# zzyunzhi/object-intrinsics

Hardware: AMD Instinct MI355X
Metric: rendered rays/sec (64x64 img, 128 samples/ray) + D-images/sec (higher is better)
Workload: dtype f32 via f16x3 (fp32 operands split into 2 fp16 limbs = 22 mantissa bits, 3 fp16 MFMAs per product, fp32 accumulate: 2^-22 relative per product, 1e-4 parity path); 1 GPU; C2: 1x64x64 crop per GPU, 64+64 samples/ray, 1 up-sampling step(s), Generator.forward (render + Phong maps) + ADADiscriminatorView forward; parallelism=dp1 (independent renders, no data-path collective)

## Files before the change

object-intrinsics_amd/build.py:

```python
import hashlib
import os
import subprocess
import sys

HERE = os.path.dirname(os.path.abspath(__file__))
CSRC = os.path.join(HERE, "csrc")
OUT_DIR = os.path.join(HERE, "oi_amd")
LIB = os.path.join(OUT_DIR, "liboi_hip.so")
STAMP = os.path.join(OUT_DIR, ".liboi_hip.stamp")
SOURCES = ["mlp.hip", "mlp_fwd3.hip", "mlp_fwd3b.hip", "color_head.hip", "render.hip", "disc.hip", "disc_small.hip", "disc_large.hip", "mlp_bwd.hip", "render_bwd.hip", "disc_bwd.hip", "optim.hip", "loss.hip", "mesh.hip", "relight.hip", "mesh_attr.hip", "trace.hip", "mesh_band.hip", "occlusion.hip", "trace_batch.hip", "envlight.hip", "scene.hip"]
FLAGS = ["--offload-arch=gfx950", "-O3", "-std=c++17", "-fPIC", "-Wno-unused-value"] + os.environ.get("OI_FLAGS", "").split()
EXTRA = {"mlp_fwd3.hip": ["-mllvm", "-amdgpu-mfma-vgpr-form=1"],
         "mlp_fwd3b.hip": ["-mllvm", "-amdgpu-mfma-vgpr-form=1", "-fno-slp-vectorize"],
         "mlp_bwd.hip": ["-mllvm", "-amdgpu-mfma-vgpr-form=1"]}


def _hipcc():
    for c in (os.environ.get("HIPCC"), "/opt/rocm/bin/hipcc", "hipcc"):
        if c and (os.path.isabs(c) and os.path.exists(c) or not os.path.isabs(c)):
            return c
    raise RuntimeError("hipcc not found")


def _sources():
    return [s for s in SOURCES if os.path.exists(os.path.join(CSRC, s))]


def _digest():
    h = hashlib.sha256()
    files = [os.path.join(CSRC, f) for f in sorted(os.listdir(CSRC))]
    inc = os.path.join(os.path.dirname(HERE), "include")
    files += [os.path.join(inc, f) for f in sorted(os.listdir(inc))]
    for f in files:
        with open(f, "rb") as fh:
            h.update(os.path.basename(f).encode())
# ... 37 lines not shown
```

object-intrinsics_amd/csrc/mlp_fwd3.hip:

```cpp
#include <type_traits>

#include "mlp_common.h"
#include "f3_blob.h"

namespace {

using namespace oimlp;
static_assert(oif3::FC == C && oif3::HB_SIG == H_SIG && oif3::HB_TABS_END == H_TABS_END && oif3::HB_BIAS == H_BIAS &&
              oif3::HB_WSCALE == H_WSCALE && oif3::HB_NL_SDF == NL_SDF, "f3_blob.h mirrors the packed header's offsets");

constexpr int F3_WAVES = 4;
constexpr int F3_TILE = F3_WAVES * WAVE_PTS;
using oif3::F3_FILM;
using oif3::F3_FILM_ROW;
using oif3::F3_TABS;
using oif3::F3_GMAX;
using oif3::F3_BLOB;
constexpr int F3_LDS = F3_BLOB + 2 * 65536;

typedef float Bank[16][4];
__device__ __forceinline__ float to_acc(float v) {
  float a;
  asm("v_accvgpr_write_b32 %0, %1" : "=a"(a) : "v"(v));
  return a;
}
__device__ __forceinline__ float from_acc(float a) {
  float v;
  asm("v_accvgpr_read_b32 %0, %1" : "=v"(v) : "a"(a));
  return v;
}

constexpr int F3_CU_SLOTS = 4096;
constexpr int F3_WG_SLOTS = 512;
__device__ __forceinline__ int cu_slot_id() {
  const unsigned xcc = __builtin_amdgcn_s_getreg((4 - 1) << 11 | 0 << 6 | 20);
  const unsigned cu = __builtin_amdgcn_s_getreg((8 - 1) << 11 | 8 << 6 | 4);
  return (int)(xcc * 256 + cu);
}

typedef float f32x2 __attribute__((ext_vector_type(2)));
__device__ __forceinline__ f32x2 pk_fma(f32x2 a, f32x2 b, f32x2 c) {
  return __builtin_elementwise_fma(a, b, c);
}
__device__ __forceinline__ f32x2 pk_mul(f32x2 a, f32x2 b) {
  return a * b;
}
__device__ __forceinline__ f32x2 pk_mul_s(f32x2 a, float s) {
  return a * s;
}
__device__ __forceinline__ f32x2 film_phase2(const f32x4& a, const f32x4& b, int k, float acc0, float acc1) {
  return pk_fma(f32x2{a[k], a[k + 1]}, f32x2{acc0, acc1}, f32x2{b[k], b[k + 1]});
}
__device__ __forceinline__ float max3_abs(float m, float x, float y) {
  float r;
  asm("v_max3_f32 %0, %1, |%2|, |%3|" : "=v"(r) : "v"(m), "v"(x), "v"(y));
  return r;
}

typedef unsigned Limbs[8][4];


__device__ __forceinline__ void split_limbs_normalised(const float (&act)[64], float m, float& run, Limbs& bh, Limbs& bl) {
  m = fmaxf(m, __shfl_xor(m, 32, 64));
  int eb = (__builtin_bit_cast(int, m) >> 23) & 0xff;
  eb = eb < 14 ? 14 : (eb > 254 ? 254 : eb);
  const float sc = __builtin_bit_cast(float, (267 - eb) << 23);
  run *= __builtin_bit_cast(float, (eb - 13) << 23);
#pragma unroll
  for (int s = 0; s < 8; ++s) {
#pragma unroll
    for (int d = 0; d < 4; ++d) split_pair(act[8 * s + 2 * d] * sc, act[8 * s + 2 * d + 1] * sc, bh[s][d], bl[s][d]);
    __builtin_amdgcn_sched_barrier(0);
  }
}
__device__ __forceinline__ void split_limbs(const float (&act)[64], Limbs& bh, Limbs& bl) {
#pragma unroll
  for (int s = 0; s < 8; ++s) {
#pragma unroll
    for (int d = 0; d < 4; ++d) split_pair(act[8 * s + 2 * d], act[8 * s + 2 * d + 1], bh[s][d], bl[s][d]);
    __builtin_amdgcn_sched_barrier(0);
  }
}

struct NoTail {
  __device__ __forceinline__ void operator()(int, int) const {}
};
template <class T> struct is_no_tail { static constexpr bool value = false; };
template <> struct is_no_tail<NoTail> { static constexpr bool value = true; };

constexpr int F3_ADIST = 1;
constexpr int F3_VALU_PER_MFMA = 6;
struct NoMid {
  __device__ __forceinline__ void operator()() const {}
};
template <class TAIL, class MID, class EPI>
__device__ __forceinline__ void stream_layer(const char* lds, const LayOff& y, const Limbs& bh, const Limbs& bl,
                                             f32x16 (&acc)[4], TAIL&& tail, MID&& mid, EPI&& epi) {
  constexpr bool HAS_TAIL = !is_no_tail<std::remove_cv_t<std::remove_reference_t<TAIL>>>::value;
  constexpr int AD = F3_ADIST;
  f32x4 ah[AD + 1], al[AD + 1];
#pragma unroll
  for (int i = 0; i < AD; ++i) {
    ah[i] = lds_f4(lds, i * 1024, y.wl);
    al[i] = lds_f4(lds, i * 1024, y.wh);
  }
#pragma unroll
  for (int t = 0; t < 4; ++t) {
#pragma unroll
    for (int r = 0; r < 16; ++r) acc[t][r] = 0.f;
#pragma unroll
    for (int s = 0; s < 8; ++s) {
      const int cur = t * 8 + s, nxt = cur + AD;
      if (nxt < 32) {
        ah[nxt % (AD + 1)] = lds_f4(lds, nxt * 1024, y.wl);
        al[nxt % (AD + 1)] = lds_f4(lds, nxt * 1024, y.wh);
      }
      int npairs = 0;
      if (t == 0) {
        if (HAS_TAIL && s < 6) {
          constexpr int first[7] = {0, 2, 3, 4, 6, 7, 8};
          for (int rp = first[s]; rp < first[s + 1]; ++rp) tail(3, rp);
          npairs = first[s + 1] - first[s];
        }
      } else {
        epi(t - 1, s);
        npairs = 1;
      }
      const int ci = cur % (AD + 1);
      const f16x8 wh = __builtin_bit_cast(f16x8, ah[ci]);
      const f16x8 wl = __builtin_bit_cast(f16x8, al[ci]);
      const u32x4 uh = {bh[s][0], bh[s][1], bh[s][2], bh[s][3]}, ul = {bl[s][0], bl[s][1], bl[s][2], bl[s][3]};
      const f16x8 vh = __builtin_bit_cast(f16x8, uh);
      const f16x8 vl = __builtin_bit_cast(f16x8, ul);
      acc[t] = __builtin_amdgcn_mfma_f32_32x32x16_f16(wl, vh, acc[t], 0, 0, 0);
      acc[t] = __builtin_amdgcn_mfma_f32_32x32x16_f16(wh, vl, acc[t], 0, 0, 0);
      acc[t] = __builtin_amdgcn_mfma_f32_32x32x16_f16(wh, vh, acc[t], 0, 0, 0);
      if (npairs >= 1) {
#pragma unroll
        for (int q = 0; q < 2; ++q) {
          __builtin_amdgcn_sched_group_barrier(0x008, 1, 0);
          if (npairs <= 1) __builtin_amdgcn_sched_group_barrier(0x002, F3_VALU_PER_MFMA, 0);
          else __builtin_amdgcn_sched_group_barrier(0x002, 2 * F3_VALU_PER_MFMA, 0);
        }
        __builtin_amdgcn_sched_group_barrier(0x008, 1, 0);
      }
      __builtin_amdgcn_sched_barrier(0);
    }
    if (t == 0) {
      mid();
      __builtin_amdgcn_sched_barrier(0);
    }
  }
}
template <class EPI>
__device__ __forceinline__ void run_tail(EPI&& epi) {
#pragma unroll
  for (int rp = 0; rp < 8; ++rp) {
    epi(3, rp);
    if (rp & 1) __builtin_amdgcn_sched_barrier(0);
  }
}

#ifdef OI_F3_PROF
__device__ unsigned long long oi_prof3[16];
#define F3_T(i)                                                  \
  do {                                                           \
    const unsigned long long t_ = __builtin_readcyclecounter();  \
    pacc[i] += t_ - tprev;                                       \
    tprev = t_;                                                  \
  } while (0)
#else
#define F3_T(i)
#endif

template <bool FAST>
__global__ void __launch_bounds__(64 * F3_WAVES) __attribute__((amdgpu_waves_per_eu(1, 1)))
sdf_mlp_full3_kernel(const float* __restrict__ pts, const char* __restrict__ packed, const float* __restrict__ gamma,
                     const float* __restrict__ beta, float* __restrict__ sdf_out, float* __restrict__ grad_out,
                     float* __restrict__ rgb_out, float* __restrict__ feat_out, char* __restrict__ scratch,
                     const char* __restrict__ blob, long long n_per_elem) {
  extern __shared__ __attribute__((aligned(16))) char lds[];
  constexpr int LB = 65536;
#ifdef OI_F3_PROF
// ... 21 lines not shown
    valid = local < n_per_elem;
    return (long long)e * n_per_elem + (valid ? local : n_per_elem - 1);
  };

  FwdScratch<false> ws;
  {
    long long wg = (long long)e * gridDim.x + blockIdx.x;
    if ((long long)gridDim.x * gridDim.y > F3_WG_SLOTS) wg = cu_slot_id();
    ws.rs = __builtin_amdgcn_make_buffer_rsrc(scratch + (wg * F3_WAVES + wave) * 16384ll, 0, 16384, 0x00020000);
  }

  __amdgpu_buffer_rsrc_t feat_rs;
  int feat_off;
  {
    const long long base_pt = (long long)e * n_per_elem + (long long)blockIdx.x * F3_TILE + wave * WAVE_PTS;
    const long long left = n_per_elem - ((long long)blockIdx.x * F3_TILE + wave * WAVE_PTS);
    const int npts = feat_out == nullptr ? 0 : (left >= WAVE_PTS ? WAVE_PTS : (left > 0 ? (int)left : 0));
    feat_rs = __builtin_amdgcn_make_buffer_rsrc(feat_out + base_pt * C, 0, npts * C * 4, 0x00020000);
    feat_off = j * C * 4 + 16 * h;
  }

  const __amdgpu_buffer_rsrc_t img_rs =
      __builtin_amdgcn_make_buffer_rsrc(const_cast<char*>(mats), 0, NMAT * LB, 0x00020000);
  auto prefetch = [&](int pos) {
    const int m = pos < 7 ? pos : (pos < 12 ? 20 - pos : (pos < 14 ? pos - 12 : (pos < 16 ? 22 - pos : 14)));
#pragma unroll
    for (int q = 0; q < LB / 4096 / F3_WAVES; ++q) {
      const int c = (wave * (LB / 4096 / F3_WAVES) + q) * 4096;
      auto* dst = (__attribute__((address_space(3))) void*)(lds + F3_BLOB + (pos & 1) * LB + c);
      __builtin_amdgcn_raw_ptr_buffer_load_lds(img_rs, dst, 16, o.l16, m * LB + c, 0, 0);
      __builtin_amdgcn_raw_ptr_buffer_load_lds(img_rs, dst, 16, o.l16, m * LB + c, 1024, 0);
      __builtin_amdgcn_raw_ptr_buffer_load_lds(img_rs, dst, 16, o.l16, m * LB + c, 2048, 0);
      __builtin_amdgcn_raw_ptr_buffer_load_lds(img_rs, dst, 16, o.l16, m * LB + c, 3072, 0);
    }
  };
  auto lay = [&](int pos) {
    LayOff y;
    y.wl = o.l16 + F3_BLOB + (pos & 1) * LB;
    y.wh = y.wl + 32768;
    y.wq = 0;
    y.f16 = 0;
    return y;
  };
  auto film_base = [&](int l) { return o.h16 + F3_FILM + l * F3_FILM_ROW; };

  float px, py, pz;
  {
    bool valid;
    const long long pt = point_of(valid);
    px = pts[pt * 3 + 0], py = pts[pt * 3 + 1], pz = pts[pt * 3 + 2];
  }
  {
    const __amdgpu_buffer_rsrc_t blob_rs =
        __builtin_amdgcn_make_buffer_rsrc(const_cast<char*>(blob + (size_t)e * F3_BLOB), 0, F3_BLOB, 0x00020000);
#pragma unroll
    for (int q = 0; q < (F3_BLOB / 1024 + F3_WAVES - 1) / F3_WAVES; ++q) {
      const int c = q * F3_WAVES + wave;
      if (c < F3_BLOB / 1024)
        __builtin_amdgcn_raw_ptr_buffer_load_lds(blob_rs, (__attribute__((address_space(3))) void*)(lds + c * 1024), 16, o.l16,
                                                 c * 1024, 0, 0);
    }
  }
  prefetch(0);
  asm volatile("s_waitcnt vmcnt(%0) lgkmcnt(0)\n\ts_barrier" ::"n"(LB / 1024 / F3_WAVES) : "memory");
#ifdef OI_F3_PROF
  unsigned long long pacc[8] = {0, 0, 0, 0, 0, 0, 0, 0};
  unsigned long long tprev = __builtin_readcyclecounter();
  const unsigned long long tstart = tprev;
  pacc[4] = tstart - t_entry;
#endif
  float act[64];
  f32x16 acc[4];
  Limbs AH, AL, BH, BL;
  Bank P0, P1, P2, P3;
  struct Rows {
    f32x4 a, b, c, d;
  } rw[2];
  f32x4 fv;
  float run = 1.f, vmax = 0.f, sdf_part = 0.f;

  auto reduce = [&](float phi) { return FAST ? phi : __builtin_amdgcn_fractf(phi); };
  auto ld = [&](int imm, int base) { return lds_f4(lds, imm, base); };
#define ROW_A(FB, G) ld(grp_f0(G) * 4, FB)
#define ROW_B(FB, G) ld((C + grp_f0(G)) * 4, FB)
#define ROW_G(FB, G) ld((2 * C + grp_f0(G)) * 4, FB)
#define ROW_SIG(G) ld(F3_TABS + (H_SIG + grp_f0(G)) * 4, o.h16)

#define OI_PARK(BANK) [&](int g, int k, float r) { BANK[g][k] = to_acc(r); }
  auto no_park = [](int, int, float) {};

  auto layer0 = [&](Limbs& NH, Limbs& NL, auto&& park) {
    const int fb = film_base(0);
#pragma unroll
    for (int g = 0; g < 16; ++g) {
      const f32x4 a4 = ROW_A(fb, g), b4 = ROW_B(fb, g);
      float sn[4];
#pragma unroll
      for (int k = 0; k < 4; ++k) {
        const f32x4 w = lds_f4(lds, F3_TABS + H_TAB0 * 4 + (grp_f0(g) + k) * 16, o.h64);
        const float u = fmaf(pz, w[2], fmaf(py, w[1], px * w[0]));
        const float r = reduce(fmaf(a4[k], u, b4[k]));
        sn[k] = __builtin_amdgcn_sinf(r);
        park(g, k, r);
      }
      split_pair(sn[0], sn[1], NH[g >> 1][2 * (g & 1)], NL[g >> 1][2 * (g & 1)]);
      split_pair(sn[2], sn[3], NH[g >> 1][2 * (g & 1) + 1], NL[g >> 1][2 * (g & 1) + 1]);
      if (g & 1) __builtin_amdgcn_sched_barrier(0);
    }
  };

#define OI_FWD_EPI(FB, NH, NL, PARK, NEXT)                                                                 \
  [&](int tb, int rp) {                                                                                    \
    const int g = tb * 4 + (rp >> 1), k = 2 * (rp & 1);                                                    \
    Rows& R = rw[g & 1];                                                                                   \
    if (k == 0) {                                                                                          \
      if (g < 15) {                                                                                        \
        rw[(g + 1) & 1].a = ROW_A(FB, g + 1);                                                              \
        rw[(g + 1) & 1].b = ROW_B(FB, g + 1);                                                              \
      } else {                                                                                             \
        NEXT;                                                                                              \
      }                                                                                                    \
    }                                                                                                      \
    const f32x2 ph = film_phase2(R.a, R.b, k, acc[tb][2 * rp], acc[tb][2 * rp + 1]);                 \
    const float r0 = reduce(ph[0]), r1 = reduce(ph[1]);                                                    \
    PARK(g, k, r0);                                                                                        \
    PARK(g, k + 1, r1);                                                                                    \
    split_pair(__builtin_amdgcn_sinf(r0), __builtin_amdgcn_sinf(r1), NH[2 * tb + (rp >> 2)][rp & 3],       \
               NL[2 * tb + (rp >> 2)][rp & 3]);                                                            \
  }
  float sg = 1.f;
  auto pow2_for = [&](float U) {
    int eb = (__builtin_bit_cast(int, U) >> 23) & 0xff;
    eb = eb < 15 ? 15 : (eb > 253 ? 253 : eb);
    run *= __builtin_bit_cast(float, (eb - 14) << 23);
    sg = __builtin_bit_cast(float, (268 - eb) << 23);
  };
  const float* gmax = reinterpret_cast<const float*>(lds + F3_GMAX);
#define OI_REV_MID(L)                                                          \
  [&]() {                                                                      \
    const float m = fmaxf(vmax, __shfl_xor(vmax, 32, 64));                     \
    pow2_for(m * (hdr[H_BOUND + 6 + (L)] * gmax[(L)-1]));                      \
    vmax = 0.f;                                                                \
  }
#define OI_REV_EPI(FB, BANK, NH, NL, NEXT)                                                                 \
  [&](int tb, int rp) {                                                                                    \
    const int g = tb * 4 + (rp >> 1), k = 2 * (rp & 1);                                                    \
    Rows& R = rw[g & 1];                                                                                   \
    if (k == 0) {                                                                                          \
      if (g < 15) {                                                                                        \
        rw[(g + 1) & 1].c = ROW_G(FB, g + 1);                                                              \
      } else {                                                                                             \
        NEXT;                                                                                              \
      }                                                                                                    \
    }                                                                                                      \
    const f32x2 cs = {__builtin_amdgcn_cosf(from_acc(BANK[g][k])), __builtin_amdgcn_cosf(from_acc(BANK[g][k + 1]))};                     \
    const f32x2 v = pk_mul(pk_mul_s(f32x2{acc[tb][2 * rp], acc[tb][2 * rp + 1]}, sg),                \
                           pk_mul(f32x2{R.c[k], R.c[k + 1]}, cs));                                         \
    vmax = max3_abs(vmax, v[0], v[1]);                                                                     \
    split_pair(v[0], v[1], NH[2 * tb + (rp >> 2)][rp & 3], NL[2 * tb + (rp >> 2)][rp & 3]);                \
  }

  const LayOff y1 = lay(0), y2 = lay(1), y3 = lay(2), y4 = lay(3), y5 = lay(4), y6 = lay(5), y7 = lay(6);
  const int F0 = film_base(0), F1 = film_base(1), F2 = film_base(2), F3 = film_base(3), F4 = film_base(4),
            F5 = film_base(5), F6 = film_base(6), F7 = film_base(7), F8 = film_base(8), F9 = film_base(9);
#define NEXT_AB(FB) (rw[0].a = ROW_A(FB, 0), rw[0].b = ROW_B(FB, 0))
#define NEXT_G(FB) (rw[0].c = ROW_G(FB, 0))

  layer0(AH, AL, no_park);
  NEXT_AB(F1);
  F3_T(0);
  ring_sync();
  F3_T(2);
  prefetch(1);
  auto park0 = OI_PARK(P0);
  auto park1 = OI_PARK(P1);
  auto park2 = OI_PARK(P2);
  auto park3 = OI_PARK(P3);
  auto e1 = OI_FWD_EPI(F1, BH, BL, no_park, NEXT_AB(F2));
  stream_layer(lds, y1, AH, AL, acc, NoTail(), NoMid(), e1);
  F3_T(1);
  ring_sync();
  F3_T(2);
  prefetch(2);
  auto e2 = OI_FWD_EPI(F2, AH, AL, no_park, NEXT_AB(F3));
  stream_layer(lds, y2, BH, BL, acc, e1, NoMid(), e2);
  F3_T(1);
  ring_sync();
  F3_T(2);
  prefetch(3);
  auto e3 = OI_FWD_EPI(F3, BH, BL, park0, NEXT_AB(F4));
  stream_layer(lds, y3, AH, AL, acc, e2, NoMid(), e3);
  F3_T(1);
  ring_sync();
  F3_T(2);
  prefetch(4);
  auto e4 = OI_FWD_EPI(F4, AH, AL, park1, NEXT_AB(F5));
  stream_layer(lds, y4, BH, BL, acc, e3, NoMid(), e4);
  F3_T(1);
  ring_sync();
  F3_T(2);
  prefetch(5);
  auto e5 = OI_FWD_EPI(F5, BH, BL, park2, NEXT_AB(F6));
  stream_layer(lds, y5, AH, AL, acc, e4, NoMid(), e5);
  F3_T(1);
  ring_sync();
  F3_T(2);
  prefetch(6);
  auto e6 = OI_FWD_EPI(F6, AH, AL, park3,
                       (NEXT_AB(F7), rw[0].c = ROW_A(F9, 0), rw[0].d = ROW_SIG(0)));
  stream_layer(lds, y6, BH, BL, acc, e5, NoMid(), e6);
  F3_T(1);
  ring_sync();
  F3_T(2);
  prefetch(7);
  pow2_for(gmax[9] * 2.0f);
  const float sg7 = sg;
  auto e7 = [&](int tb, int rp) {
    const int g = tb * 4 + (rp >> 1), k = 2 * (rp & 1);
    Rows& R = rw[g & 1];
    if (k == 0) {
      if (g < 15) {
        Rows& N = rw[(g + 1) & 1];
        N.a = ROW_A(F7, g + 1);
        N.b = ROW_B(F7, g + 1);
        N.c = ROW_A(F9, g + 1);
        N.d = ROW_SIG(g + 1);
      } else {
        NEXT_G(F6);
      }
    }
    const f32x2 ph = film_phase2(R.a, R.b, k, acc[tb][2 * rp], acc[tb][2 * rp + 1]);
    f32x2 cs;
#pragma unroll
    for (int i = 0; i < 2; ++i) {
      const float r = reduce(ph[i]);
      const float sn = __builtin_amdgcn_sinf(r);
      fv[k + i] = sn;
      sdf_part = fmaf(sn, R.d[k + i], sdf_part);
      cs[i] = __builtin_amdgcn_cosf(r);
    }
    const f32x2 v = pk_mul(pk_mul_s(f32x2{R.c[k], R.c[k + 1]}, sg7), cs);
    vmax = max3_abs(vmax, v[0], v[1]);
    split_pair(v[0], v[1], BH[2 * tb + (rp >> 2)][rp & 3], BL[2 * tb + (rp >> 2)][rp & 3]);
    if (k == 2) {
      ws.store(0, g, o, fv);
      __builtin_amdgcn_raw_buffer_store_b128(__builtin_bit_cast(u32x4, fv), feat_rs, feat_off + grp_f0(g) * 4, 0, 0);
    }
  };
  stream_layer(lds, y7, AH, AL, acc, e6, NoMid(), e7);
  F3_T(1);
  ring_sync();
  F3_T(2);
  prefetch(8);

  auto r7 = OI_REV_EPI(F6, P3, AH, AL, NEXT_G(F5));
  stream_layer(lds, lay(7), BH, BL, acc, e7, OI_REV_MID(7), r7);
  {
    sdf_part += __shfl_xor(sdf_part, 32, 64);
    const float sdf_v = sdf_part + *reinterpret_cast<const float*>(lds + F3_TABS + (H_SIG + C) * 4);
    bool valid;
    const long long pt = point_of(valid);
    if (valid && h == 0) sdf_out[pt] = sdf_v;
  }
  F3_T(1);
  ring_sync();
  F3_T(2);
  prefetch(9);
  auto r6 = OI_REV_EPI(F5, P2, BH, BL, NEXT_G(F4));
  stream_layer(lds, lay(8), AH, AL, acc, r7, OI_REV_MID(6), r6);
  F3_T(1);
  ring_sync();
  F3_T(2);
  prefetch(10);
  auto r5 = OI_REV_EPI(F4, P1, AH, AL, NEXT_G(F3));
  stream_layer(lds, lay(9), BH, BL, acc, r6, OI_REV_MID(5), r5);
  F3_T(1);
  ring_sync();
  F3_T(2);
  prefetch(11);
  auto r4 = OI_REV_EPI(F3, P0, BH, BL, (void)0);
  stream_layer(lds, lay(10), AH, AL, acc, r5, OI_REV_MID(4), r4);
  F3_T(1);
  ring_sync();
  F3_T(2);
  prefetch(12);
  float one = 1.0f;
  asm volatile("" : "+v"(one));
  auto pg3 = [&](int tb, int rp) {
    const int g = tb * 4 + (rp >> 1), k = 2 * (rp & 1);
    const f32x2 a = pk_mul_s(f32x2{acc[tb][2 * rp], acc[tb][2 * rp + 1]}, one);
    vmax = max3_abs(vmax, a[0], a[1]);
    P0[g][k] = to_acc(a[0]);
    P0[g][k + 1] = to_acc(a[1]);
  };
  stream_layer(lds, lay(11), BH, BL, acc, r4, [&]() { vmax = 0.f; }, pg3);
  F3_T(1);
  ring_sync();
  F3_T(2);
  prefetch(13);
  run_tail(pg3);
  F3_T(3);

  const LayOff z1 = lay(12), z2 = lay(13);
  NEXT_AB(F1);
  layer0(AH, AL, park1);
  F3_T(0);
  auto f1 = OI_FWD_EPI(F1, BH, BL, park2, (NEXT_AB(F2), NEXT_G(F2)));
  stream_layer(lds, z1, AH, AL, acc, NoTail(), NoMid(), f1);
  F3_T(1);
  ring_sync();
  F3_T(2);
  prefetch(14);
  pow2_for(fmaxf(vmax, __shfl_xor(vmax, 32, 64)) * gmax[2]);
  vmax = 0.f;
  const float sg2 = sg;
  auto f2 = [&](int tb, int rp) {
    const int g = tb * 4 + (rp >> 1), k = 2 * (rp & 1);
    Rows& R = rw[g & 1];
    if (k == 0) {
      if (g < 15) {
        Rows& N = rw[(g + 1) & 1];
        N.a = ROW_A(F2, g + 1);
        N.b = ROW_B(F2, g + 1);
        N.c = ROW_G(F2, g + 1);
      } else {
        NEXT_G(F1);
      }
    }
    const f32x2 ph = film_phase2(R.a, R.b, k, acc[tb][2 * rp], acc[tb][2 * rp + 1]);
    const f32x2 cs = {__builtin_amdgcn_cosf(reduce(ph[0])), __builtin_amdgcn_cosf(reduce(ph[1]))};
    const f32x2 v = pk_mul(pk_mul_s(f32x2{from_acc(P0[g][k]), from_acc(P0[g][k + 1])}, sg2), pk_mul(f32x2{R.c[k], R.c[k + 1]}, cs));
    vmax = max3_abs(vmax, v[0], v[1]);
    split_pair(v[0], v[1], AH[2 * tb + (rp >> 2)][rp & 3], AL[2 * tb + (rp >> 2)][rp & 3]);
  };
  stream_layer(lds, z2, BH, BL, acc, f1, NoMid(), f2);
  F3_T(1);
  ring_sync();
  F3_T(2);
  prefetch(15);

  auto r2 = OI_REV_EPI(F1, P2, BH, BL, NEXT_G(F0));
  stream_layer(lds, lay(14), AH, AL, acc, f2, OI_REV_MID(2), r2);
  F3_T(1);
  ring_sync();
  F3_T(2);
  prefetch(16);
  auto r1 = [&](int tb, int rp) {
    const int g = tb * 4 + (rp >> 1), k = 2 * (rp & 1);
    Rows& R = rw[g & 1];
    if (k == 0 && g < 15) rw[(g + 1) & 1].c = ROW_G(F0, g + 1);
    const f32x2 cs = {__builtin_amdgcn_cosf(from_acc(P1[g][k])), __builtin_amdgcn_cosf(from_acc(P1[g][k + 1]))};
    const f32x2 v = pk_mul(f32x2{acc[tb][2 * rp], acc[tb][2 * rp + 1]}, pk_mul(f32x2{R.c[k], R.c[k + 1]}, cs));
    act[4 * g + k] = v[0];
    act[4 * g + k + 1] = v[1];
  };
  stream_layer(lds, lay(15), BH, BL, acc, r2, [&]() {}, r1);
  F3_T(1);
  run_tail(r1);
  F3_T(3);
  f32x4 fback[16];
#pragma unroll
  for (int g = 0; g < 16; ++g) fback[g] = ws.load(0, g, o);
  float gx = 0.f, gy = 0.f, gz = 0.f;
#pragma unroll
  for (int g = 0; g < 16; ++g) {
#pragma unroll
    for (int k = 0; k < 4; ++k) {
      const f32x4 w = lds_f4(lds, F3_TABS + H_TAB0 * 4 + (grp_f0(g) + k) * 16, o.h64);
      const float v = act[4 * g + k];
      gx = fmaf(v, w[0], gx);
      gy = fmaf(v, w[1], gy);
      gz = fmaf(v, w[2], gz);
    }
    if (g & 1) __builtin_amdgcn_sched_barrier(0);
  }
  gx += __shfl_xor(gx, 32, 64);
  gy += __shfl_xor(gy, 32, 64);
  gz += __shfl_xor(gz, 32, 64);
  gx *= run;
  gy *= run;
  gz *= run;
  bool valid;
  const long long pt = point_of(valid);
  if (valid && h == 0) {
    grad_out[pt * 3 + 0] = gx;
    grad_out[pt * 3 + 1] = gy;
    grad_out[pt * 3 + 2] = gz;
  }

  {
    ring_sync();
#pragma unroll
    for (int g = 0; g < 16; ++g)
#pragma unroll
      for (int k = 0; k < 4; ++k) act[4 * g + k] = fback[g][k];
    const LayOff yc = lay(16);
    const float cs3 = 1.0f / hdr[H_WSCALE + 14];
    const float vx = gx * cs3, vy = gy * cs3, vz = gz * cs3;
    float r0 = 0.f, r1 = 0.f, r2 = 0.f;
    f32x4 w0, w1, w2;
    split_limbs(act, AH, AL);
    NEXT_AB(F8);
    auto ec = [&](int tb, int rp) {
      const int g = tb * 4 + (rp >> 1), k = 2 * (rp & 1);
      Rows& R = rw[g & 1];
      if (k == 0) {
        if (g < 15) {
          rw[(g + 1) & 1].a = ROW_A(F8, g + 1);
          rw[(g + 1) & 1].b = ROW_B(F8, g + 1);
        }
        w0 = lds_f4(lds, F3_TABS + (H_RGB + 0 * C + grp_f0(g)) * 4, o.h16);
        w1 = lds_f4(lds, F3_TABS + (H_RGB + 1 * C + grp_f0(g)) * 4, o.h16);
        w2 = lds_f4(lds, F3_TABS + (H_RGB + 2 * C + grp_f0(g)) * 4, o.h16);
      }
#pragma unroll
      for (int i = 0; i < 2; ++i) {
        const f32x4 w = lds_f4(lds, F3_TABS + H_TABV * 4 + (grp_f0(g) + k + i) * 16, o.h64);
        const float u = acc[tb][2 * rp + i] + fmaf(vz, w[2], fmaf(vy, w[1], vx * w[0]));
        const float sn = __builtin_amdgcn_sinf(reduce(fmaf(R.a[k + i], u, R.b[k + i])));
        r0 = fmaf(sn, w0[k + i], r0);
        r1 = fmaf(sn, w1[k + i], r1);
        r2 = fmaf(sn, w2[k + i], r2);
      }
    };
    F3_T(5);
    stream_layer(lds, yc, AH, AL, acc, NoTail(), NoMid(), ec);
    F3_T(1);
    run_tail(ec);
    F3_T(3);
    r0 += __shfl_xor(r0, 32, 64);
    r1 += __shfl_xor(r1, 32, 64);
    r2 += __shfl_xor(r2, 32, 64);
    if (valid && h == 0 && rgb_out != nullptr) {
      const float* brgb = reinterpret_cast<const float*>(lds + F3_TABS + (H_RGB + 3 * C) * 4);
      rgb_out[pt * 3 + 0] = oi::sigmoidf_(r0 + brgb[0]);
      rgb_out[pt * 3 + 1] = oi::sigmoidf_(r1 + brgb[1]);
      rgb_out[pt * 3 + 2] = oi::sigmoidf_(r2 + brgb[2]);
    }
  }
#ifdef OI_F3_PROF
  F3_T(5);
  if (lane == 0) {
    for (int i = 0; i < 6; ++i) atomicAdd(&oi_prof3[i], pacc[i]);
    atomicAdd(&oi_prof3[6], __builtin_readcyclecounter() - tstart);
    atomicAdd(&oi_prof3[7], 1ull);
    atomicAdd(&oi_prof3[8], __builtin_readcyclecounter() - t_entry);
    atomicAdd(&oi_prof3[9], __builtin_amdgcn_s_memrealtime() - rt_entry);
  }
#endif
#undef OI_PARK
#undef OI_FWD_EPI
#undef OI_REV_EPI
#undef OI_REV_MID
#undef NEXT_AB
#undef NEXT_G
#undef ROW_A
#undef ROW_B
#undef ROW_G
#undef ROW_SIG
}

__global__ void __launch_bounds__(128) film_blob_f3_kernel(const char* __restrict__ packed, const float* __restrict__ gamma,
                                                           const float* __restrict__ beta, char* __restrict__ blob) {
  __shared__ float red[8];
  const int e = blockIdx.x, l = blockIdx.y, tid = threadIdx.x;
  const float* hdr = reinterpret_cast<const float*>(packed);
  float* out = reinterpret_cast<float*>(blob + (size_t)e * F3_BLOB);
  const float gm = tid < C ? gamma[((size_t)e * 9 + l) * C + tid] : 0.f, bt = tid < C ? beta[((size_t)e * 9 + l) * C + tid] : 0.f;
  oif3::blob_layer(hdr, out, l, tid, gm, bt, red);
}

size_t full3_slot_bytes(int B, long long n_per_elem) {
  const long long wgs = (long long)B * oi::cdiv(n_per_elem, F3_TILE);
// ... 78 lines not shown
```

Measured before the change: 3.556 million rays/s.

## Interleave weight DMA and split epilogues into MFMA gaps in fused SIREN kernel

Each layer's epilogue is split into three phases that run between the three fp16 MFMAs of every step, replacing sched_group_barrier hints with explicit sched barriers. The next layer's weight prefetch is broken into 16 pieces issued one per MFMA step inside stream_layer, instead of one burst before each layer. Packed f32x2 math is replaced by scalar fmas, SLP vectorization is disabled for this file, and point coordinates are reloaded before the second pass. The aim is to hide VALU and DMA issue behind matrix ops, at the cost of more live state (st[]) and tighter scheduling constraints.

```diff
diff --git a/object-intrinsics_amd/build.py b/object-intrinsics_amd/build.py
--- a/object-intrinsics_amd/build.py
+++ b/object-intrinsics_amd/build.py
@@ -10,7 +10,7 @@
 STAMP = os.path.join(OUT_DIR, ".liboi_hip.stamp")
 SOURCES = ["mlp.hip", "mlp_fwd3.hip", "mlp_fwd3b.hip", "color_head.hip", "render.hip", "disc.hip", "disc_small.hip", "disc_large.hip", "mlp_bwd.hip", "render_bwd.hip", "disc_bwd.hip", "optim.hip", "loss.hip", "mesh.hip", "relight.hip", "mesh_attr.hip", "trace.hip", "mesh_band.hip", "occlusion.hip", "trace_batch.hip", "envlight.hip", "scene.hip"]
 FLAGS = ["--offload-arch=gfx950", "-O3", "-std=c++17", "-fPIC", "-Wno-unused-value"] + os.environ.get("OI_FLAGS", "").split()
-EXTRA = {"mlp_fwd3.hip": ["-mllvm", "-amdgpu-mfma-vgpr-form=1"],
+EXTRA = {"mlp_fwd3.hip": ["-mllvm", "-amdgpu-mfma-vgpr-form=1", "-fno-slp-vectorize"],
          "mlp_fwd3b.hip": ["-mllvm", "-amdgpu-mfma-vgpr-form=1", "-fno-slp-vectorize"],
          "mlp_bwd.hip": ["-mllvm", "-amdgpu-mfma-vgpr-form=1"]}
 
diff --git a/object-intrinsics_amd/csrc/mlp_fwd3.hip b/object-intrinsics_amd/csrc/mlp_fwd3.hip
--- a/object-intrinsics_amd/csrc/mlp_fwd3.hip
+++ b/object-intrinsics_amd/csrc/mlp_fwd3.hip
@@ -38,18 +38,11 @@
   return (int)(xcc * 256 + cu);
 }
 
-typedef float f32x2 __attribute__((ext_vector_type(2)));
-__device__ __forceinline__ f32x2 pk_fma(f32x2 a, f32x2 b, f32x2 c) {
-  return __builtin_elementwise_fma(a, b, c);
-}
-__device__ __forceinline__ f32x2 pk_mul(f32x2 a, f32x2 b) {
-  return a * b;
-}
-__device__ __forceinline__ f32x2 pk_mul_s(f32x2 a, float s) {
-  return a * s;
-}
-__device__ __forceinline__ f32x2 film_phase2(const f32x4& a, const f32x4& b, int k, float acc0, float acc1) {
-  return pk_fma(f32x2{a[k], a[k + 1]}, f32x2{acc0, acc1}, f32x2{b[k], b[k + 1]});
+struct Pair2 {
+  float x, y;
+};
+__device__ __forceinline__ Pair2 film_phase2(const f32x4& a, const f32x4& b, int k, float acc0, float acc1) {
+  return Pair2{fmaf(a[k], acc0, b[k]), fmaf(a[k + 1], acc1, b[k + 1])};
 }
 __device__ __forceinline__ float max3_abs(float m, float x, float y) {
   float r;
@@ -83,19 +76,22 @@
 }
 
 struct NoTail {
-  __device__ __forceinline__ void operator()(int, int) const {}
+  __device__ __forceinline__ void operator()(int, int, int) const {}
 };
 template <class T> struct is_no_tail { static constexpr bool value = false; };
 template <> struct is_no_tail<NoTail> { static constexpr bool value = true; };
 
 constexpr int F3_ADIST = 1;
-constexpr int F3_VALU_PER_MFMA = 6;
+constexpr int F3_DMA_PIECES = 16;
 struct NoMid {
   __device__ __forceinline__ void operator()() const {}
 };
-template <class TAIL, class MID, class EPI>
+struct NoDma {
+  __device__ __forceinline__ void operator()(int) const {}
+};
+template <class TAIL, class MID, class EPI, class DMA>
 __device__ __forceinline__ void stream_layer(const char* lds, const LayOff& y, const Limbs& bh, const Limbs& bl,
-                                             f32x16 (&acc)[4], TAIL&& tail, MID&& mid, EPI&& epi) {
+                                             f32x16 (&acc)[4], TAIL&& tail, MID&& mid, EPI&& epi, DMA&& dma) {
   constexpr bool HAS_TAIL = !is_no_tail<std::remove_cv_t<std::remove_reference_t<TAIL>>>::value;
   constexpr int AD = F3_ADIST;
   f32x4 ah[AD + 1], al[AD + 1];
@@ -111,21 +107,18 @@
 #pragma unroll
     for (int s = 0; s < 8; ++s) {
       const int cur = t * 8 + s, nxt = cur + AD;
-      if (nxt < 32) {
-        ah[nxt % (AD + 1)] = lds_f4(lds, nxt * 1024, y.wl);
-        al[nxt % (AD + 1)] = lds_f4(lds, nxt * 1024, y.wh);
-      }
-      int npairs = 0;
-      if (t == 0) {
-        if (HAS_TAIL && s < 6) {
-          constexpr int first[7] = {0, 2, 3, 4, 6, 7, 8};
-          for (int rp = first[s]; rp < first[s + 1]; ++rp) tail(3, rp);
-          npairs = first[s + 1] - first[s];
+      auto gap = [&](int q) {
+        if (t == 0) {
+          if (HAS_TAIL && s == 0) {
+            tail(3, (2 * q) / 3, (2 * q) % 3);
+            tail(3, (2 * q + 1) / 3, (2 * q + 1) % 3);
+          } else if (HAS_TAIL && s < 7) {
+            tail(3, s + 1, q);
+          }
+        } else {
+          epi(t - 1, s, q);
         }
-      } else {
-        epi(t - 1, s);
-        npairs = 1;
-      }
+      };
       const int ci = cur % (AD + 1);
       const f16x8 wh = __builtin_bit_cast(f16x8, ah[ci]);
       const f16x8 wl = __builtin_bit_cast(f16x8, al[ci]);
@@ -133,17 +126,18 @@
       const f16x8 vh = __builtin_bit_cast(f16x8, uh);
       const f16x8 vl = __builtin_bit_cast(f16x8, ul);
       acc[t] = __builtin_amdgcn_mfma_f32_32x32x16_f16(wl, vh, acc[t], 0, 0, 0);
+      if (nxt < 32) {
+        ah[nxt % (AD + 1)] = lds_f4(lds, nxt * 1024, y.wl);
+        al[nxt % (AD + 1)] = lds_f4(lds, nxt * 1024, y.wh);
+      }
+      gap(0);
+      __builtin_amdgcn_sched_barrier(0);
       acc[t] = __builtin_amdgcn_mfma_f32_32x32x16_f16(wh, vl, acc[t], 0, 0, 0);
+      if (cur < F3_DMA_PIECES) dma(cur);
+      gap(1);
+      __builtin_amdgcn_sched_barrier(0);
       acc[t] = __builtin_amdgcn_mfma_f32_32x32x16_f16(wh, vh, acc[t], 0, 0, 0);
-      if (npairs >= 1) {
-#pragma unroll
-        for (int q = 0; q < 2; ++q) {
-          __builtin_amdgcn_sched_group_barrier(0x008, 1, 0);
-          if (npairs <= 1) __builtin_amdgcn_sched_group_barrier(0x002, F3_VALU_PER_MFMA, 0);
-          else __builtin_amdgcn_sched_group_barrier(0x002, 2 * F3_VALU_PER_MFMA, 0);
-        }
-        __builtin_amdgcn_sched_group_barrier(0x008, 1, 0);
-      }
+      gap(2);
       __builtin_amdgcn_sched_barrier(0);
     }
     if (t == 0) {
@@ -154,11 +148,14 @@
 }
 template <class EPI>
 __device__ __forceinline__ void run_tail(EPI&& epi) {
+  asm volatile("; oi-exposed-begin");
 #pragma unroll
   for (int rp = 0; rp < 8; ++rp) {
-    epi(3, rp);
+#pragma unroll
+    for (int q = 0; q < 3; ++q) epi(3, rp, q);
     if (rp & 1) __builtin_amdgcn_sched_barrier(0);
   }
+  asm volatile("; oi-exposed-end");
 }
 
 #ifdef OI_F3_PROF
@@ -226,24 +223,31 @@
 
   const __amdgpu_buffer_rsrc_t img_rs =
       __builtin_amdgcn_make_buffer_rsrc(const_cast<char*>(mats), 0, NMAT * LB, 0x00020000);
+  constexpr int F3_PIECES = LB / 1024 / F3_WAVES;
+  static_assert(F3_PIECES == F3_DMA_PIECES, "stream_layer issues every piece of a wave's share");
+  auto prefetch_piece = [&](int pos, int i) {
+    const int m = pos < 7 ? pos : (pos < 12 ? 20 - pos : (pos < 14 ? pos - 12 : (pos < 16 ? 22 - pos : 14)));
+    const int c = (wave * (F3_PIECES / 4) + i / 4) * 4096;
+    auto* dst = (__attribute__((address_space(3))) void*)(lds + F3_BLOB + (pos & 1) * LB + c);
+    switch (i % 4) {
+      case 0: __builtin_amdgcn_raw_ptr_buffer_load_lds(img_rs, dst, 16, o.l16, m * LB + c, 0, 0); break;
+      case 1: __builtin_amdgcn_raw_ptr_buffer_load_lds(img_rs, dst, 16, o.l16, m * LB + c, 1024, 0); break;
+      case 2: __builtin_amdgcn_raw_ptr_buffer_load_lds(img_rs, dst, 16, o.l16, m * LB + c, 2048, 0); break;
+      default: __builtin_amdgcn_raw_ptr_buffer_load_lds(img_rs, dst, 16, o.l16, m * LB + c, 3072, 0); break;
+    }
+  };
   auto prefetch = [&](int pos) {
-    const int m = pos < 7 ? pos : (pos < 12 ? 20 - pos : (pos < 14 ? pos - 12 : (pos < 16 ? 22 - pos : 14)));
-#pragma unroll
-    for (int q = 0; q < LB / 4096 / F3_WAVES; ++q) {
-      const int c = (wave * (LB / 4096 / F3_WAVES) + q) * 4096;
-      auto* dst = (__attribute__((address_space(3))) void*)(lds + F3_BLOB + (pos & 1) * LB + c);
-      __builtin_amdgcn_raw_ptr_buffer_load_lds(img_rs, dst, 16, o.l16, m * LB + c, 0, 0);
-      __builtin_amdgcn_raw_ptr_buffer_load_lds(img_rs, dst, 16, o.l16, m * LB + c, 1024, 0);
-      __builtin_amdgcn_raw_ptr_buffer_load_lds(img_rs, dst, 16, o.l16, m * LB + c, 2048, 0);
-      __builtin_amdgcn_raw_ptr_buffer_load_lds(img_rs, dst, 16, o.l16, m * LB + c, 3072, 0);
-    }
-  };
+#pragma unroll
+    for (int i = 0; i < F3_PIECES; ++i) prefetch_piece(pos, i);
+  };
+#define OI_DMA(POS) [&](int i) { prefetch_piece(POS, i); }
   auto lay = [&](int pos) {
     LayOff y;
     y.wl = o.l16 + F3_BLOB + (pos & 1) * LB;
     y.wh = y.wl + 32768;
     y.wq = 0;
     y.f16 = 0;
+    asm volatile("" : "+v"(y.wl), "+v"(y.wh));
     return y;
   };
   auto film_base = [&](int l) { return o.h16 + F3_FILM + l * F3_FILM_ROW; };
@@ -282,6 +286,7 @@
   } rw[2];
   f32x4 fv;
   float run = 1.f, vmax = 0.f, sdf_part = 0.f;
+  float st[6];
 
   auto reduce = [&](float phi) { return FAST ? phi : __builtin_amdgcn_fractf(phi); };
   auto ld = [&](int imm, int base) { return lds_f4(lds, imm, base); };
@@ -314,23 +319,29 @@
   };
 
 #define OI_FWD_EPI(FB, NH, NL, PARK, NEXT)                                                                 \
-  [&](int tb, int rp) {                                                                                    \
+  [&](int tb, int rp, int q) {                                                                             \
     const int g = tb * 4 + (rp >> 1), k = 2 * (rp & 1);                                                    \
     Rows& R = rw[g & 1];                                                                                   \
-    if (k == 0) {                                                                                          \
-      if (g < 15) {                                                                                        \
-        rw[(g + 1) & 1].a = ROW_A(FB, g + 1);                                                              \
-        rw[(g + 1) & 1].b = ROW_B(FB, g + 1);                                                              \
-      } else {                                                                                             \
-        NEXT;                                                                                              \
+    if (q == 0) {                                                                                          \
+      const Pair2 ph = film_phase2(R.a, R.b, k, acc[tb][2 * rp], acc[tb][2 * rp + 1]);                     \
+      st[0] = reduce(ph.x);                                                                                \
+      st[1] = reduce(ph.y);                                                                                \
+    } else if (q == 1) {                                                                                   \
+      if (k == 0) {                                                                                        \
+        if (g < 15) {                                                                                      \
+          rw[(g + 1) & 1].a = ROW_A(FB, g + 1);                                                            \
+          rw[(g + 1) & 1].b = ROW_B(FB, g + 1);                                                            \
+        } else {                                                                                           \
+          NEXT;                                                                                            \
+        }                                                                                                  \
       }                                                                                                    \
+      st[2] = __builtin_amdgcn_sinf(st[0]);                                                                \
+      PARK(g, k, st[0]);                                                                                   \
+      PARK(g, k + 1, st[1]);                                                                               \
+    } else {                                                                                               \
+      split_pair(st[2], __builtin_amdgcn_sinf(st[1]), NH[2 * tb + (rp >> 2)][rp & 3],                      \
+                 NL[2 * tb + (rp >> 2)][rp & 3]);                                                          \
     }                                                                                                      \
-    const f32x2 ph = film_phase2(R.a, R.b, k, acc[tb][2 * rp], acc[tb][2 * rp + 1]);                 \
-    const float r0 = reduce(ph[0]), r1 = reduce(ph[1]);                                                    \
-    PARK(g, k, r0);                                                                                        \
-    PARK(g, k + 1, r1);                                                                                    \
-    split_pair(__builtin_amdgcn_sinf(r0), __builtin_amdgcn_sinf(r1), NH[2 * tb + (rp >> 2)][rp & 3],       \
-               NL[2 * tb + (rp >> 2)][rp & 3]);                                                            \
   }
   float sg = 1.f;
   auto pow2_for = [&](float U) {
@@ -347,24 +358,30 @@
     vmax = 0.f;                                                                \
   }
 #define OI_REV_EPI(FB, BANK, NH, NL, NEXT)                                                                 \
-  [&](int tb, int rp) {                                                                                    \
+  [&](int tb, int rp, int q) {                                                                             \
     const int g = tb * 4 + (rp >> 1), k = 2 * (rp & 1);                                                    \
     Rows& R = rw[g & 1];                                                                                   \
-    if (k == 0) {                                                                                          \
-      if (g < 15) {                                                                                        \
-        rw[(g + 1) & 1].c = ROW_G(FB, g + 1);                                                              \
-      } else {                                                                                             \
-        NEXT;                                                                                              \
+    if (q == 0) {                                                                                          \
+      st[0] = __builtin_amdgcn_cosf(from_acc(BANK[g][k]));                                                 \
+      st[1] = from_acc(BANK[g][k + 1]);                                                                    \
+    } else if (q == 1) {                                                                                   \
+      if (k == 0) {                                                                                        \
+        if (g < 15) {                                                                                      \
+          rw[(g + 1) & 1].c = ROW_G(FB, g + 1);                                                            \
+        } else {                                                                                           \
+          NEXT;                                                                                            \
+        }                                                                                                  \
       }                                                                                                    \
+      st[2] = __builtin_amdgcn_cosf(st[1]);                                                                \
+      st[3] = (acc[tb][2 * rp] * sg) * (R.c[k] * st[0]);                                                   \
+      st[4] = acc[tb][2 * rp + 1] * sg;                                                                    \
+    } else {                                                                                               \
+      const float v1 = st[4] * (R.c[k + 1] * st[2]);                                                       \
+      vmax = max3_abs(vmax, st[3], v1);                                                                    \
+      split_pair(st[3], v1, NH[2 * tb + (rp >> 2)][rp & 3], NL[2 * tb + (rp >> 2)][rp & 3]);               \
     }                                                                                                      \
-    const f32x2 cs = {__builtin_amdgcn_cosf(from_acc(BANK[g][k])), __builtin_amdgcn_cosf(from_acc(BANK[g][k + 1]))};                     \
-    const f32x2 v = pk_mul(pk_mul_s(f32x2{acc[tb][2 * rp], acc[tb][2 * rp + 1]}, sg),                \
-                           pk_mul(f32x2{R.c[k], R.c[k + 1]}, cs));                                         \
-    vmax = max3_abs(vmax, v[0], v[1]);                                                                     \
-    split_pair(v[0], v[1], NH[2 * tb + (rp >> 2)][rp & 3], NL[2 * tb + (rp >> 2)][rp & 3]);                \
-  }
-
-  const LayOff y1 = lay(0), y2 = lay(1), y3 = lay(2), y4 = lay(3), y5 = lay(4), y6 = lay(5), y7 = lay(6);
+  }
+
   const int F0 = film_base(0), F1 = film_base(1), F2 = film_base(2), F3 = film_base(3), F4 = film_base(4),
             F5 = film_base(5), F6 = film_base(6), F7 = film_base(7), F8 = film_base(8), F9 = film_base(9);
 #define NEXT_AB(FB) (rw[0].a = ROW_A(FB, 0), rw[0].b = ROW_B(FB, 0))
@@ -375,90 +392,88 @@
   F3_T(0);
   ring_sync();
   F3_T(2);
-  prefetch(1);
   auto park0 = OI_PARK(P0);
   auto park1 = OI_PARK(P1);
   auto park2 = OI_PARK(P2);
   auto park3 = OI_PARK(P3);
   auto e1 = OI_FWD_EPI(F1, BH, BL, no_park, NEXT_AB(F2));
-  stream_layer(lds, y1, AH, AL, acc, NoTail(), NoMid(), e1);
-  F3_T(1);
-  ring_sync();
-  F3_T(2);
-  prefetch(2);
+  stream_layer(lds, lay(0), AH, AL, acc, NoTail(), NoMid(), e1, OI_DMA(1));
+  F3_T(1);
+  ring_sync();
+  F3_T(2);
   auto e2 = OI_FWD_EPI(F2, AH, AL, no_park, NEXT_AB(F3));
-  stream_layer(lds, y2, BH, BL, acc, e1, NoMid(), e2);
-  F3_T(1);
-  ring_sync();
-  F3_T(2);
-  prefetch(3);
+  stream_layer(lds, lay(1), BH, BL, acc, e1, NoMid(), e2, OI_DMA(2));
+  F3_T(1);
+  ring_sync();
+  F3_T(2);
   auto e3 = OI_FWD_EPI(F3, BH, BL, park0, NEXT_AB(F4));
-  stream_layer(lds, y3, AH, AL, acc, e2, NoMid(), e3);
-  F3_T(1);
-  ring_sync();
-  F3_T(2);
-  prefetch(4);
+  stream_layer(lds, lay(2), AH, AL, acc, e2, NoMid(), e3, OI_DMA(3));
+  F3_T(1);
+  ring_sync();
+  F3_T(2);
   auto e4 = OI_FWD_EPI(F4, AH, AL, park1, NEXT_AB(F5));
-  stream_layer(lds, y4, BH, BL, acc, e3, NoMid(), e4);
-  F3_T(1);
-  ring_sync();
-  F3_T(2);
-  prefetch(5);
+  stream_layer(lds, lay(3), BH, BL, acc, e3, NoMid(), e4, OI_DMA(4));
+  F3_T(1);
+  ring_sync();
+  F3_T(2);
   auto e5 = OI_FWD_EPI(F5, BH, BL, park2, NEXT_AB(F6));
-  stream_layer(lds, y5, AH, AL, acc, e4, NoMid(), e5);
-  F3_T(1);
-  ring_sync();
-  F3_T(2);
-  prefetch(6);
+  stream_layer(lds, lay(4), AH, AL, acc, e4, NoMid(), e5, OI_DMA(5));
+  F3_T(1);
+  ring_sync();
+  F3_T(2);
   auto e6 = OI_FWD_EPI(F6, AH, AL, park3,
                        (NEXT_AB(F7), rw[0].c = ROW_A(F9, 0), rw[0].d = ROW_SIG(0)));
-  stream_layer(lds, y6, BH, BL, acc, e5, NoMid(), e6);
-  F3_T(1);
-  ring_sync();
-  F3_T(2);
-  prefetch(7);
+  stream_layer(lds, lay(5), BH, BL, acc, e5, NoMid(), e6, OI_DMA(6));
+  F3_T(1);
+  ring_sync();
+  F3_T(2);
   pow2_for(gmax[9] * 2.0f);
   const float sg7 = sg;
-  auto e7 = [&](int tb, int rp) {
+  auto e7 = [&](int tb, int rp, int q) {
     const int g = tb * 4 + (rp >> 1), k = 2 * (rp & 1);
     Rows& R = rw[g & 1];
-    if (k == 0) {
-      if (g < 15) {
-        Rows& N = rw[(g + 1) & 1];
-        N.a = ROW_A(F7, g + 1);
-        N.b = ROW_B(F7, g + 1);
-        N.c = ROW_A(F9, g + 1);
-        N.d = ROW_SIG(g + 1);
-      } else {
-        NEXT_G(F6);
+    if (q == 0) {
+      const Pair2 ph = film_phase2(R.a, R.b, k, acc[tb][2 * rp], acc[tb][2 * rp + 1]);
+      st[0] = reduce(ph.x);
+      st[1] = reduce(ph.y);
+      st[2] = __builtin_amdgcn_sinf(st[0]);
+    } else if (q == 1) {
+      if (k == 0) {
+        if (g < 15) {
+          Rows& N = rw[(g + 1) & 1];
+          N.a = ROW_A(F7, g + 1);
+          N.b = ROW_B(F7, g + 1);
+          N.c = ROW_A(F9, g + 1);
+          N.d = ROW_SIG(g + 1);
+        } else {
+          NEXT_G(F6);
+        }
       }
-    }
-    const f32x2 ph = film_phase2(R.a, R.b, k, acc[tb][2 * rp], acc[tb][2 * rp + 1]);
-    f32x2 cs;
-#pragma unroll
-    for (int i = 0; i < 2; ++i) {
-      const float r = reduce(ph[i]);
-      const float sn = __builtin_amdgcn_sinf(r);
-      fv[k + i] = sn;
-      sdf_part = fmaf(sn, R.d[k + i], sdf_part);
-      cs[i] = __builtin_amdgcn_cosf(r);
-    }
-    const f32x2 v = pk_mul(pk_mul_s(f32x2{R.c[k], R.c[k + 1]}, sg7), cs);
-    vmax = max3_abs(vmax, v[0], v[1]);
-    split_pair(v[0], v[1], BH[2 * tb + (rp >> 2)][rp & 3], BL[2 * tb + (rp >> 2)][rp & 3]);
-    if (k == 2) {
-      ws.store(0, g, o, fv);
-      __builtin_amdgcn_raw_buffer_store_b128(__builtin_bit_cast(u32x4, fv), feat_rs, feat_off + grp_f0(g) * 4, 0, 0);
-    }
-  };
-  stream_layer(lds, y7, AH, AL, acc, e6, NoMid(), e7);
-  F3_T(1);
-  ring_sync();
-  F3_T(2);
-  prefetch(8);
+      fv[k] = st[2];
+      sdf_part = fmaf(st[2], R.d[k], sdf_part);
+      asm volatile("" : "+v"(sdf_part));
+      st[3] = (R.c[k] * sg7) * __builtin_amdgcn_cosf(st[0]);
+      st[4] = __builtin_amdgcn_sinf(st[1]);
+    } else {
+      fv[k + 1] = st[4];
+      sdf_part = fmaf(st[4], R.d[k + 1], sdf_part);
+      asm volatile("" : "+v"(sdf_part));
+      const float v1 = (R.c[k + 1] * sg7) * __builtin_amdgcn_cosf(st[1]);
+      vmax = max3_abs(vmax, st[3], v1);
+      split_pair(st[3], v1, BH[2 * tb + (rp >> 2)][rp & 3], BL[2 * tb + (rp >> 2)][rp & 3]);
+      if (k == 2) {
+        ws.store(0, g, o, fv);
+        __builtin_amdgcn_raw_buffer_store_b128(__builtin_bit_cast(u32x4, fv), feat_rs, feat_off + grp_f0(g) * 4, 0, 0);
+      }
+    }
+  };
+  stream_layer(lds, lay(6), AH, AL, acc, e6, NoMid(), e7, OI_DMA(7));
+  F3_T(1);
+  ring_sync();
+  F3_T(2);
 
   auto r7 = OI_REV_EPI(F6, P3, AH, AL, NEXT_G(F5));
-  stream_layer(lds, lay(7), BH, BL, acc, e7, OI_REV_MID(7), r7);
+  stream_layer(lds, lay(7), BH, BL, acc, e7, OI_REV_MID(7), r7, OI_DMA(8));
   {
     sdf_part += __shfl_xor(sdf_part, 32, 64);
     const float sdf_v = sdf_part + *reinterpret_cast<const float*>(lds + F3_TABS + (H_SIG + C) * 4);
@@ -469,96 +484,109 @@
   F3_T(1);
   ring_sync();
   F3_T(2);
-  prefetch(9);
   auto r6 = OI_REV_EPI(F5, P2, BH, BL, NEXT_G(F4));
-  stream_layer(lds, lay(8), AH, AL, acc, r7, OI_REV_MID(6), r6);
-  F3_T(1);
-  ring_sync();
-  F3_T(2);
-  prefetch(10);
+  stream_layer(lds, lay(8), AH, AL, acc, r7, OI_REV_MID(6), r6, OI_DMA(9));
+  F3_T(1);
+  ring_sync();
+  F3_T(2);
   auto r5 = OI_REV_EPI(F4, P1, AH, AL, NEXT_G(F3));
-  stream_layer(lds, lay(9), BH, BL, acc, r6, OI_REV_MID(5), r5);
-  F3_T(1);
-  ring_sync();
-  F3_T(2);
-  prefetch(11);
+  stream_layer(lds, lay(9), BH, BL, acc, r6, OI_REV_MID(5), r5, OI_DMA(10));
+  F3_T(1);
+  ring_sync();
+  F3_T(2);
   auto r4 = OI_REV_EPI(F3, P0, BH, BL, (void)0);
-  stream_layer(lds, lay(10), AH, AL, acc, r5, OI_REV_MID(4), r4);
-  F3_T(1);
-  ring_sync();
-  F3_T(2);
-  prefetch(12);
+  stream_layer(lds, lay(10), AH, AL, acc, r5, OI_REV_MID(4), r4, OI_DMA(11));
+  F3_T(1);
+  ring_sync();
+  F3_T(2);
   float one = 1.0f;
   asm volatile("" : "+v"(one));
-  auto pg3 = [&](int tb, int rp) {
+  auto pg3 = [&](int tb, int rp, int q) {
     const int g = tb * 4 + (rp >> 1), k = 2 * (rp & 1);
-    const f32x2 a = pk_mul_s(f32x2{acc[tb][2 * rp], acc[tb][2 * rp + 1]}, one);
-    vmax = max3_abs(vmax, a[0], a[1]);
-    P0[g][k] = to_acc(a[0]);
-    P0[g][k + 1] = to_acc(a[1]);
-  };
-  stream_layer(lds, lay(11), BH, BL, acc, r4, [&]() { vmax = 0.f; }, pg3);
-  F3_T(1);
-  ring_sync();
-  F3_T(2);
-  prefetch(13);
+    if (q == 0) {
+      st[0] = acc[tb][2 * rp] * one;
+      st[1] = acc[tb][2 * rp + 1] * one;
+    } else if (q == 1) {
+      vmax = max3_abs(vmax, st[0], st[1]);
+      P0[g][k] = to_acc(st[0]);
+    } else {
+      P0[g][k + 1] = to_acc(st[1]);
+    }
+  };
+  stream_layer(lds, lay(11), BH, BL, acc, r4, [&]() { vmax = 0.f; }, pg3, OI_DMA(12));
+  F3_T(1);
+  ring_sync();
+  F3_T(2);
   run_tail(pg3);
   F3_T(3);
 
-  const LayOff z1 = lay(12), z2 = lay(13);
   NEXT_AB(F1);
+  {
+    bool valid;
+    const long long pt = point_of(valid);
+    px = pts[pt * 3 + 0], py = pts[pt * 3 + 1], pz = pts[pt * 3 + 2];
+  }
   layer0(AH, AL, park1);
   F3_T(0);
   auto f1 = OI_FWD_EPI(F1, BH, BL, park2, (NEXT_AB(F2), NEXT_G(F2)));
-  stream_layer(lds, z1, AH, AL, acc, NoTail(), NoMid(), f1);
-  F3_T(1);
-  ring_sync();
-  F3_T(2);
-  prefetch(14);
+  stream_layer(lds, lay(12), AH, AL, acc, NoTail(), NoMid(), f1, OI_DMA(13));
+  F3_T(1);
+  ring_sync();
+  F3_T(2);
   pow2_for(fmaxf(vmax, __shfl_xor(vmax, 32, 64)) * gmax[2]);
   vmax = 0.f;
   const float sg2 = sg;
-  auto f2 = [&](int tb, int rp) {
+  auto f2 = [&](int tb, int rp, int q) {
     const int g = tb * 4 + (rp >> 1), k = 2 * (rp & 1);
     Rows& R = rw[g & 1];
-    if (k == 0) {
-      if (g < 15) {
-        Rows& N = rw[(g + 1) & 1];
-        N.a = ROW_A(F2, g + 1);
-        N.b = ROW_B(F2, g + 1);
-        N.c = ROW_G(F2, g + 1);
-      } else {
-        NEXT_G(F1);
+    if (q == 0) {
+      const Pair2 ph = film_phase2(R.a, R.b, k, acc[tb][2 * rp], acc[tb][2 * rp + 1]);
+      st[0] = reduce(ph.x);
+      st[1] = reduce(ph.y);
+    } else if (q == 1) {
+      if (k == 0) {
+        if (g < 15) {
+          Rows& N = rw[(g + 1) & 1];
+          N.a = ROW_A(F2, g + 1);
+          N.b = ROW_B(F2, g + 1);
+          N.c = ROW_G(F2, g + 1);
+        } else {
+          NEXT_G(F1);
+        }
       }
-    }
-    const f32x2 ph = film_phase2(R.a, R.b, k, acc[tb][2 * rp], acc[tb][2 * rp + 1]);
-    const f32x2 cs = {__builtin_amdgcn_cosf(reduce(ph[0])), __builtin_amdgcn_cosf(reduce(ph[1]))};
-    const f32x2 v = pk_mul(pk_mul_s(f32x2{from_acc(P0[g][k]), from_acc(P0[g][k + 1])}, sg2), pk_mul(f32x2{R.c[k], R.c[k + 1]}, cs));
-    vmax = max3_abs(vmax, v[0], v[1]);
-    split_pair(v[0], v[1], AH[2 * tb + (rp >> 2)][rp & 3], AL[2 * tb + (rp >> 2)][rp & 3]);
-  };
-  stream_layer(lds, z2, BH, BL, acc, f1, NoMid(), f2);
-  F3_T(1);
-  ring_sync();
-  F3_T(2);
-  prefetch(15);
+      st[3] = (from_acc(P0[g][k]) * sg2) * (R.c[k] * __builtin_amdgcn_cosf(st[0]));
+      st[4] = from_acc(P0[g][k + 1]) * sg2;
+    } else {
+      const float v1 = st[4] * (R.c[k + 1] * __builtin_amdgcn_cosf(st[1]));
+      vmax = max3_abs(vmax, st[3], v1);
+      split_pair(st[3], v1, AH[2 * tb + (rp >> 2)][rp & 3], AL[2 * tb + (rp >> 2)][rp & 3]);
+    }
+  };
+  stream_layer(lds, lay(13), BH, BL, acc, f1, NoMid(), f2, OI_DMA(14));
+  F3_T(1);
+  ring_sync();
+  F3_T(2);
 
   auto r2 = OI_REV_EPI(F1, P2, BH, BL, NEXT_G(F0));
-  stream_layer(lds, lay(14), AH, AL, acc, f2, OI_REV_MID(2), r2);
-  F3_T(1);
-  ring_sync();
-  F3_T(2);
-  prefetch(16);
-  auto r1 = [&](int tb, int rp) {
+  stream_layer(lds, lay(14), AH, AL, acc, f2, OI_REV_MID(2), r2, OI_DMA(15));
+  F3_T(1);
+  ring_sync();
+  F3_T(2);
+  auto r1 = [&](int tb, int rp, int q) {
     const int g = tb * 4 + (rp >> 1), k = 2 * (rp & 1);
     Rows& R = rw[g & 1];
-    if (k == 0 && g < 15) rw[(g + 1) & 1].c = ROW_G(F0, g + 1);
-    const f32x2 cs = {__builtin_amdgcn_cosf(from_acc(P1[g][k])), __builtin_amdgcn_cosf(from_acc(P1[g][k + 1]))};
-    const f32x2 v = pk_mul(f32x2{acc[tb][2 * rp], acc[tb][2 * rp + 1]}, pk_mul(f32x2{R.c[k], R.c[k + 1]}, cs));
-    act[4 * g + k] = v[0];
-    act[4 * g + k + 1] = v[1];
-  };
-  stream_layer(lds, lay(15), BH, BL, acc, r2, [&]() {}, r1);
+    if (q == 0) {
+      st[0] = __builtin_amdgcn_cosf(from_acc(P1[g][k]));
+      st[1] = from_acc(P1[g][k + 1]);
+    } else if (q == 1) {
+      if (k == 0 && g < 15) rw[(g + 1) & 1].c = ROW_G(F0, g + 1);
+      st[2] = __builtin_amdgcn_cosf(st[1]);
+      act[4 * g + k] = acc[tb][2 * rp] * (R.c[k] * st[0]);
+    } else {
+      act[4 * g + k + 1] = acc[tb][2 * rp + 1] * (R.c[k + 1] * st[2]);
+    }
+  };
+  stream_layer(lds, lay(15), BH, BL, acc, r2, [&]() {}, r1, OI_DMA(16));
   F3_T(1);
   run_tail(r1);
   F3_T(3);
@@ -598,37 +626,48 @@
     for (int g = 0; g < 16; ++g)
 #pragma unroll
       for (int k = 0; k < 4; ++k) act[4 * g + k] = fback[g][k];
-    const LayOff yc = lay(16);
     const float cs3 = 1.0f / hdr[H_WSCALE + 14];
     const float vx = gx * cs3, vy = gy * cs3, vz = gz * cs3;
     float r0 = 0.f, r1 = 0.f, r2 = 0.f;
     f32x4 w0, w1, w2;
     split_limbs(act, AH, AL);
     NEXT_AB(F8);
-    auto ec = [&](int tb, int rp) {
+    f32x4 tv[2];
+    auto ec = [&](int tb, int rp, int q) {
       const int g = tb * 4 + (rp >> 1), k = 2 * (rp & 1);
       Rows& R = rw[g & 1];
-      if (k == 0) {
-        if (g < 15) {
-          rw[(g + 1) & 1].a = ROW_A(F8, g + 1);
-          rw[(g + 1) & 1].b = ROW_B(F8, g + 1);
-        }
-        w0 = lds_f4(lds, F3_TABS + (H_RGB + 0 * C + grp_f0(g)) * 4, o.h16);
-        w1 = lds_f4(lds, F3_TABS + (H_RGB + 1 * C + grp_f0(g)) * 4, o.h16);
-        w2 = lds_f4(lds, F3_TABS + (H_RGB + 2 * C + grp_f0(g)) * 4, o.h16);
-      }
-#pragma unroll
-      for (int i = 0; i < 2; ++i) {
-        const f32x4 w = lds_f4(lds, F3_TABS + H_TABV * 4 + (grp_f0(g) + k + i) * 16, o.h64);
-        const float u = acc[tb][2 * rp + i] + fmaf(vz, w[2], fmaf(vy, w[1], vx * w[0]));
-        const float sn = __builtin_amdgcn_sinf(reduce(fmaf(R.a[k + i], u, R.b[k + i])));
+      auto inner = [&](int i) { return fmaf(vz, tv[i][2], fmaf(vy, tv[i][1], vx * tv[i][0])); };
+      auto sine = [&](int i, float in) {
+        const float u = acc[tb][2 * rp + i] + in;
+        return __builtin_amdgcn_sinf(reduce(fmaf(R.a[k + i], u, R.b[k + i])));
+      };
+      auto sum = [&](int i, float sn) {
         r0 = fmaf(sn, w0[k + i], r0);
         r1 = fmaf(sn, w1[k + i], r1);
         r2 = fmaf(sn, w2[k + i], r2);
+      };
+      if (q == 0) {
+        if (k == 0) {
+          if (g < 15) {
+            rw[(g + 1) & 1].a = ROW_A(F8, g + 1);
+            rw[(g + 1) & 1].b = ROW_B(F8, g + 1);
+          }
+          w0 = lds_f4(lds, F3_TABS + (H_RGB + 0 * C + grp_f0(g)) * 4, o.h16);
+          w1 = lds_f4(lds, F3_TABS + (H_RGB + 1 * C + grp_f0(g)) * 4, o.h16);
+          w2 = lds_f4(lds, F3_TABS + (H_RGB + 2 * C + grp_f0(g)) * 4, o.h16);
+        }
+        tv[0] = lds_f4(lds, F3_TABS + H_TABV * 4 + (grp_f0(g) + k) * 16, o.h64);
+        tv[1] = lds_f4(lds, F3_TABS + H_TABV * 4 + (grp_f0(g) + k + 1) * 16, o.h64);
+      } else if (q == 1) {
+        st[0] = sine(0, inner(0));
+        st[1] = inner(1);
+      } else {
+        sum(0, st[0]);
+        sum(1, sine(1, st[1]));
       }
     };
     F3_T(5);
-    stream_layer(lds, yc, AH, AL, acc, NoTail(), NoMid(), ec);
+    stream_layer(lds, lay(16), AH, AL, acc, NoTail(), NoMid(), ec, NoDma());
     F3_T(1);
     run_tail(ec);
     F3_T(3);
@@ -653,6 +692,7 @@
   }
 #endif
 #undef OI_PARK
+#undef OI_DMA
 #undef OI_FWD_EPI
 #undef OI_REV_EPI
 #undef OI_REV_MID
```

Result: faster. 3.756 million rays/s (median of 6 runs) (+5.6%).
